# oxli-bio/oxli

Measured on NVIDIA B200. Metric: canonical k-mers counted/sec, higher is better.
Workload: dtype u64

## Files before the change

### oxli_b200/csrc/capi.cu

```cuda
#include <algorithm>
#include <atomic>
#include <cerrno>
#include <chrono>
#include <cmath>
#include <cstdarg>
#include <cstddef>
#include <condition_variable>
#include <cstdio>
#include <cstdlib>
#include <cstring>
#include <deque>
#include <functional>
#include <memory>
#include <mutex>
#include <string>
#include <system_error>
#include <thread>
#include <vector>

#include <fcntl.h>
#include <unistd.h>

#include <cuda_runtime.h>
#include <nvtx3/nvToolsExt.h>
// ... 205 lines not shown

constexpr uint64_t kScratchMin = 1024;

oxg_status ensure_io(DeviceCtx *c, uint64_t n) {
    CU(c->d_io.reserve(n, kScratchMin));
    CU(c->h_io.reserve(n, kScratchMin));
    return OXG_OK;
}

int grid_for(const DeviceCtx *c, uint64_t items, int threads, int per_sm) {
    uint64_t want = (items + threads - 1) / threads;
    return (int)std::max<uint64_t>(1, std::min<uint64_t>(want, (uint64_t)c->sms * per_sm));
}

constexpr uint64_t kSparseBytes = 128ull << 20;
uint64_t capacity_for_keys(uint64_t keys);
bool over_loaded(uint64_t size, uint64_t cap) {
    if (cap * 16 < kSparseBytes) return size * 10 > cap * 3;
    return size * 10 > cap * 7;
}

uint64_t pow2_at_least(uint64_t x) {
    uint64_t c = kMinCap;
    while (c < x) c <<= 1;
    return c;
}

uint64_t capacity_for_keys(uint64_t keys) {
    uint64_t cap = pow2_at_least(keys + keys / 2 + 1);
    while (cap * 16 < kSparseBytes && keys * 10 > cap * 3) cap <<= 1;
    return cap;
}

uint64_t slots_for(uint64_t keys) { return std::max(capacity_for_keys(keys), pow2_at_least(keys * 2)); }

oxg_status free_device_bytes(size_t *free_b) {
    size_t total = 0;
    CU(cudaMemGetInfo(free_b, &total));
    return OXG_OK;
}

oxg_status larger_and_fits(uint64_t keys, uint64_t cap, bool *yes) {
    *yes = false;
    const uint64_t want = slots_for(keys);
    if (want <= cap) return OXG_OK;
    size_t free_b = 0;
    TRY(free_device_bytes(&free_b));
    *yes = want * 16 < free_b / 2;
    return OXG_OK;
}


}

namespace {
struct PartPlan {
    uint32_t n_parts = 0, part_bits = 0;
    int n_ranks = 1, self_rank = 0, owner_shift = 64;
    uint32_t grid_a = 0;
    uint32_t frag_cap = 0;
    uint32_t batch_tiles = 1;
    uint64_t spill_cap = 0;
    uint32_t groups = 1;
    uint32_t n_dest() const { return n_parts * (uint32_t)n_ranks; }
    uint64_t frag_entries() const { return (uint64_t)n_dest() * grid_a * frag_cap; }
};

}

struct oxg_table {
    DeviceCtx *ctx = nullptr;
    uint32_t k = 0;
    DeviceArray<ulonglong2> slots;
    DeviceArray<Ctrl> d_ctrl;
    PinnedArray<Ctrl> h_ctrl;
    uint64_t size = 0;
    bool hinted = false;
    uint64_t hint_keys = 0;
    bool pooled = false;
    float last_ms_a = 0.f, last_ms_b = 0.f;
    struct {
        bool active = false;
        PartPlan pl;
        uint32_t launches = 0;
        uint64_t windows = 0, planned = 0;
    } pend;
    uint64_t part_budget = 0;
    uint32_t group_cap = 0;
    DeviceArray<uint32_t> d_sketch;
    PinnedArray<uint32_t> h_sketch;
    uint64_t sketch_covers = 0;
    uint64_t est_keys = 0;
    uint64_t last_made = 0;
    uint64_t last_new = 0;
    float last_ms = 0.f;
    uint64_t last_launches = 0;
};

namespace {

TableView view_of(const oxg_table *t, const DeferLists *defer = nullptr) {
    TableView v;
    v.slots = t->slots.get();
    v.cap = t->slots.cap();
    uint32_t lg = 0;
    while ((1ull << lg) < t->slots.cap()) ++lg;
    v.shift = 64 - lg;
    v.limit = t->slots.cap() - t->slots.cap() / 5;
    v.ctrl = t->d_ctrl.get();
    v.overflow = defer ? defer->pairs.get() : nullptr;
    v.overflow_cap = defer ? defer->pairs.cap() : 0;
    return v;
}

oxg_status pull_ctrl(oxg_table *t) {
    DeviceCtx *c = t->ctx;
    CU(cudaMemcpyAsync(t->h_ctrl.get(), t->d_ctrl.get(), sizeof(Ctrl), cudaMemcpyDeviceToHost, c->stream));
    CU(cudaStreamSynchronize(c->stream));
    t->size = t->h_ctrl.get()->size;
    return OXG_OK;
}

oxg_status zero_ctrl_fields(oxg_table *t, size_t first_field, size_t n_fields) {
    CU(cudaMemsetAsync(reinterpret_cast<uint64_t *>(t->d_ctrl.get()) + first_field, 0, n_fields * 8, t->ctx->stream));
    return OXG_OK;
}
constexpr size_t kFieldCounted = offsetof(Ctrl, counted) / 8;
constexpr size_t kFieldTile = offsetof(Ctrl, tile_counter) / 8;
constexpr size_t kLaunchFields = (offsetof(Ctrl, scratch) - offsetof(Ctrl, counted)) / 8;
constexpr size_t kFieldScratch = offsetof(Ctrl, scratch) / 8;

oxg_status alloc_slots(const oxg_table *t, uint64_t cap, DeviceArray<ulonglong2> *out) {
    DeviceCtx *c = t->ctx;
    if (t->pooled) *out = DeviceArray<ulonglong2>(c->stream);
    CU(out->reserve(cap));
    init_slots_kernel<<<grid_for(c, cap, kOpThreads, 16), kOpThreads, 0, c->stream>>>(out->get(), cap);
    LAUNCHED();
    CU(cudaGetLastError());
    return OXG_OK;
}

oxg_status grow_to_fit(oxg_table *t, uint64_t keys) {
    const uint64_t want = slots_for(keys);
    if (want <= t->slots.cap()) return OXG_OK;
    DeviceCtx *c = t->ctx;
    DeviceArray<ulonglong2> old;
    TRY(alloc_slots(t, want, &old));
    std::swap(t->slots, old);
    if (t->size) {
        rehash_kernel<<<grid_for(c, old.cap(), kOpThreads, 16), kOpThreads, 0, c->stream>>>(old.get(), old.cap(), view_of(t));
        LAUNCHED();
        CU(cudaGetLastError());
    }
    CU(cudaStreamSynchronize(c->stream));
    return OXG_OK;
}

oxg_status reserve_keys(oxg_table *t, uint64_t extra) { return grow_to_fit(t, t->size + extra); }

template <class Rebuild, class SideDrops>
oxg_status rebuild_slots(oxg_table *t, const Rebuild &rebuild, const SideDrops &side_drops, uint64_t *removed) {
    DeviceArray<ulonglong2> old;
    TRY(alloc_slots(t, t->slots.cap(), &old));
    std::swap(t->slots, old);
    rebuild(old.get());
    LAUNCHED();
    CU(cudaGetLastError());
    TRY(pull_ctrl(t));
    old.reset();
    Ctrl *h = t->h_ctrl.get();
    uint64_t n = h->scratch[0];
    h->size -= n;
    if (h->side_present && side_drops(h->side_count)) { h->side_present = 0; h->side_count = 0; ++n; }
    t->size = h->size;
    CU(cudaMemcpyAsync(t->d_ctrl.get(), h, offsetof(Ctrl, counted), cudaMemcpyHostToDevice, t->ctx->stream));
    CU(cudaStreamSynchronize(t->ctx->stream));
    if (removed) *removed = n;
    return OXG_OK;
}

oxg_status drain_deferred(oxg_table *t, DeferLists &d, uint64_t ov) {
    NvtxRange range("oxg:replay deferred");
    DeviceCtx *c = t->ctx;
    if (ov > d.pairs.cap()) return fail(OXG_ERR_CUDA, "internal: overflow list overrun");
    uint64_t prev = ~0ULL;
    while (ov) {
        const uint64_t room = std::min<uint64_t>(ov, std::max<uint64_t>(t->size, 1ull << 20));
        const uint64_t cap_before = t->slots.cap();
        TRY(grow_to_fit(t, t->size + room));
        const bool last = t->slots.cap() == cap_before && ov >= prev;
        if (last) TRY(grow_to_fit(t, t->size + ov));
        prev = ov;
        if (!last) {
            if (!d.fixed) CU(d.pairs2.reserve(ov, kScratchMin));
            else if (d.pairs2.cap() < ov) return fail(OXG_ERR_NOMEM, "deferral list too small for the replay");
        }
        TRY(zero_ctrl_fields(t, offsetof(Ctrl, overflow) / 8, 1));
        TableView v = view_of(t);
        if (!last) { v.overflow = d.pairs2.get(); v.overflow_cap = d.pairs2.cap(); }
        replay_pairs_kernel<<<grid_for(c, (ov + 3) / 4, kOpThreads, 8), kOpThreads, 0, c->stream>>>(v, d.pairs.get(), ov);
        LAUNCHED();
        CU(cudaGetLastError());
        TRY(pull_ctrl(t));
        ov = t->h_ctrl.get()->overflow;
        std::swap(d.pairs, d.pairs2);
    }
    return OXG_OK;
}

struct Counting { float ms = 0.f; uint64_t made = 0, ov = 0; };
oxg_status end_counting(oxg_table *t, uint64_t launches, uint64_t *counted, Counting *out) {
    DeviceCtx *c = t->ctx;
    CU(cudaEventRecord(c->ev_t1, c->stream));
    const uint64_t size_before = t->size;
    TRY(pull_ctrl(t));
    CU(cudaEventElapsedTime(&out->ms, c->ev_t0, c->ev_t1));
    t->last_ms += out->ms; t->last_launches += launches;
    if (counted) *counted += t->h_ctrl.get()->counted;
    out->made = t->size - size_before;
    out->ov = t->h_ctrl.get()->overflow;
    return OXG_OK;
}

#define OXG_DECLARE_ENTRY(KK) extern "C" const void *oxg_consume_entry_##KK(int mode);
OXG_FOR_EACH_K(OXG_DECLARE_ENTRY)
#undef OXG_DECLARE_ENTRY
const void *specialised_entry(uint32_t k, int mode) {
    switch (k) {
#define OXG_K_ENTRY(KK) case KK: return oxg_consume_entry_##KK(mode);
        OXG_FOR_EACH_K(OXG_K_ENTRY)
#undef OXG_K_ENTRY
    default:
        return nullptr;
    }
}
bool specialised_k(uint32_t k) { return specialised_entry(k, kModeCount) != nullptr; }
uint32_t tile_width(uint32_t k) { return specialised_k(k) ? kWarpTile : kTileW; }

oxg_status max_dyn_smem(const void *fn, int dev, size_t bytes) {
    static std::mutex mu;
    static std::vector<std::pair<const void *, int>> done;
    std::lock_guard<std::mutex> lk(mu);
    const std::pair<const void *, int> key{fn, dev};
    if (std::find(done.begin(), done.end(), key) != done.end()) return OXG_OK;
    CU(cudaFuncSetAttribute(fn, cudaFuncAttributeMaxDynamicSharedMemorySize, (int)bytes));
    done.push_back(key);
    return OXG_OK;
}

template <int MODE>
oxg_status launch_consume(oxg_table *t, const ConsumeParams &p) {
    DeviceCtx *c = t->ctx;
    const int k = (int)t->k;
    auto grid_of = [&](const void *fn, size_t smem) {
        int per_sm = 1;
        if (cudaOccupancyMaxActiveBlocksPerMultiprocessor(&per_sm, fn, kThreads, smem) != cudaSuccess || per_sm < 1) per_sm = 1;
        const uint64_t tiles_per_cta = specialised_k(t->k) ? kThreads / 32 : 1;
        const uint64_t work = p.n_tiles;
        return (int)std::max<uint64_t>(1, std::min<uint64_t>((work + tiles_per_cta - 1) / tiles_per_cta, (uint64_t)c->sms * per_sm));
    };
    if (const void *fn = specialised_entry(t->k, MODE)) {
        const size_t dyn = consume_dyn_smem(MODE);
        if (dyn) TRY(max_dyn_smem(fn, c->dev, dyn));
        void *args[] = {const_cast<ConsumeParams *>(&p)};
        CU(cudaLaunchKernel(fn, dim3(grid_of(fn, dyn)), dim3(kThreads), args, dyn, c->stream));
    } else {
        const size_t smem = generic_smem_bytes(k);
        consume_generic_kernel<MODE><<<grid_of((const void *)consume_generic_kernel<MODE>, smem), kThreads, smem, c->stream>>>(p);
    }
    LAUNCHED();
    CU(cudaGetLastError());
    return OXG_OK;
}



uint32_t group_launches(const oxg_table *t) {
    const uint32_t g = g_accumulate.load();
    return t->group_cap ? std::min(g, t->group_cap) : g;
}

bool use_partitioned(const oxg_table *t, uint64_t span) {
    if (!specialised_entry(t->k, kModePart)) return false;
    const int choice = g_pipeline.load();
    if (choice == 1) return false;
    if (choice == 2) return true;
    if (t->pend.active) return true;
    return span >= kPartMinWindows;
}

uint32_t choose_parts(const oxg_table *t, uint32_t max_parts) {
    const uint32_t forced = g_parts_override.load();
    if (forced >= 2 && !(forced & (forced - 1))) return std::min(forced, std::max(max_parts, 2u));
    const uint64_t est = std::max(t->size + t->last_new, t->hint_keys);
    if (est == 0) return std::min<uint32_t>(1024, max_parts);
    uint64_t parts = 64;
    while (parts < max_parts && parts * 6144 < est) parts <<= 1;
    return (uint32_t)std::min<uint64_t>(parts, max_parts);
}

size_t scatter_smem_rt(uint32_t k, uint32_t n_dest, uint32_t batch_tiles) {
    const uint32_t q = 8 * ((k + 7 + 7) / 8);
    const uint32_t bl = ((kWarpTile - 8 + q) + 15) / 16 * 16;
    return scatter_smem_bytes(n_dest, batch_tiles, (int)(2 * bl + 128));
}

uint64_t scatter_full_grid_tiles(const DeviceCtx *c) { return (uint64_t)c->sms * kScatCtasPerSm * kScatWarps; }
uint32_t scatter_grid(const DeviceCtx *c, uint64_t n_tiles) {
    return (uint32_t)std::max<uint64_t>(1, std::min<uint64_t>((n_tiles + kScatWarps - 1) / kScatWarps, (uint64_t)c->sms * kScatCtasPerSm));
}

oxg_status plan_partitioned(oxg_table *t, uint64_t span, uint64_t n_tiles, int n_ranks, int self_rank, PartPlan *out) {
    DeviceCtx *c = t->ctx;
    PartPlan pl;
    pl.n_parts = choose_parts(t, std::max(2u, 2048u / (uint32_t)n_ranks));
    while ((1u << pl.part_bits) < pl.n_parts) ++pl.part_bits;
    pl.n_ranks = n_ranks; pl.self_rank = self_rank;
    int lg = 0;
    while ((1 << lg) < n_ranks) ++lg;
    pl.owner_shift = 64 - lg;
    pl.batch_tiles = kScatMaxBatchTiles;
    while (pl.batch_tiles > 1 && scatter_smem_rt(t->k, pl.n_dest(), pl.batch_tiles) * kScatCtasPerSm > 220u * 1024) --pl.batch_tiles;
    if (scatter_smem_rt(t->k, pl.n_dest(), pl.batch_tiles) * kScatCtasPerSm > 220u * 1024) return fail(OXG_ERR_INVALID, "internal: too many scatter destinations");
    pl.grid_a = scatter_grid(c, n_tiles);
    if (pl.grid_a * (uint64_t)kMaxSources > kAggMaxFrags) return fail(OXG_ERR_INVALID, "internal: more pass A CTAs than pass B can take");
    const uint64_t fair = span / ((uint64_t)pl.n_dest() * pl.grid_a) + 1;
    uint64_t sq = 1;
    while (sq * sq < fair) ++sq;
    pl.frag_cap = (uint32_t)((fair + fair / 2 + 4 * sq + 3) & ~(uint64_t)3);
    pl.spill_cap = span;
    const uint32_t forced_groups = g_groups_override.load();
    pl.groups = forced_groups ? forced_groups : std::max<uint32_t>(1, std::min<uint32_t>(8, (4u * (uint32_t)c->sms + pl.n_parts - 1) / pl.n_parts));
    if (pl.frag_entries() >> 32) return fail(OXG_ERR_INVALID, "internal: fragment buffer too large for one launch");
    *out = pl;
    return OXG_OK;
}

oxg_status scatter_attr(DeviceCtx *c, uint32_t k) { return max_dyn_smem(specialised_entry(k, kModePart), c->dev, 227 * 1024); }

oxg_status ensure_part_buffers(DeviceCtx *c, const PartPlan &pl) {
    CU(c->d_frag.reserve(pl.frag_entries(), kScratchMin));
    CU(c->d_frag_cnt.reserve((uint64_t)pl.n_dest() * pl.grid_a, kScratchMin));
    CU(c->d_spill.reserve(pl.spill_cap, kScratchMin));
    CU(c->d_spill_n.reserve(1));
    return OXG_OK;
}

oxg_status launch_part_a(oxg_table *t, ConsumeParams p, const PartPlan &pl, uint64_t *d_frag, uint32_t *d_frag_cnt,
                         uint64_t *d_spill, unsigned long long *d_spill_n, cudaStream_t stream, bool append = false) {
    DeviceCtx *c = t->ctx;
    const void *fn = specialised_entry(t->k, kModePart);
    TRY(scatter_attr(c, t->k));
    const size_t dyn = scatter_smem_rt(t->k, pl.n_dest(), pl.batch_tiles);
    p.frag = d_frag; p.frag_cnt = d_frag_cnt; p.frag_cap = pl.frag_cap;
    p.n_parts = pl.n_parts; p.part_shift = 64 - pl.part_bits; p.n_dest = pl.n_dest(); p.batch_tiles = pl.batch_tiles;
    p.n_ranks = pl.n_ranks; p.self_rank = pl.self_rank; p.owner_shift = pl.owner_shift;
    p.spill = d_spill; p.spill_cap = pl.spill_cap; p.spill_n = d_spill_n;
    p.frag_append = append ? 1u : 0u;
    if (p.n_tiles >> 31) return fail(OXG_ERR_INVALID, "internal: too many tiles for one pass A launch");
    if (!append) CU(cudaMemsetAsync(d_spill_n, 0, 8, stream));
    void *args[] = {&p};
    CU(cudaLaunchKernel(fn, dim3(pl.grid_a), dim3(kScatThreads), args, dyn, stream));
    LAUNCHED();
    CU(cudaGetLastError());
    return OXG_OK;
}

constexpr int kAggThreadsDirect = 1024;
const void *const kAggCached = (const void *)aggregate_kernel<kAggThreadsDefault, true>;
const void *const kAggDirect = (const void *)aggregate_kernel<kAggThreadsDirect, false>;

uint32_t use_cache_for(const oxg_table *t, const PartPlan &pl, uint64_t windows) {
    const uint64_t keys = std::max(std::max(t->size, t->hint_keys), t->est_keys);
    return keys == 0 || (windows >= 2 * keys && keys <= 8192ull * pl.n_parts) ? 1u : 0u;
}

uint32_t aggregate_groups(const PartPlan &pl, uint32_t use_cache, uint64_t hashes) {
    if (use_cache || g_groups_override.load()) return pl.groups;
    const uint64_t items = std::max<uint64_t>(1, hashes / 40960);
    return (uint32_t)std::max<uint64_t>(pl.groups, std::min<uint64_t>(64, (items + pl.n_parts - 1) / pl.n_parts));
}

AggParams agg_params(const TableView &v, const PartPlan &pl, const AggSource *src, int n_src) {
    AggParams a{};
    a.table = v;
    for (int s = 0; s < n_src; ++s) a.src[s] = src[s];
    a.n_src = n_src;
    a.n_parts = pl.n_parts; a.dest0 = (uint32_t)pl.self_rank * pl.n_parts; a.n_ctas = pl.grid_a;
    a.frag_cap = pl.frag_cap; a.part_bits = pl.part_bits; a.spill_cap = pl.spill_cap;
    a.owner_shift = pl.owner_shift; a.self_rank = pl.self_rank; a.n_ranks = pl.n_ranks;
    return a;
}

oxg_status launch_part_b(oxg_table *t, const TableView &v, const PartPlan &pl, const AggSource *src, int n_src,
                         uint64_t windows, cudaStream_t stream) {
    DeviceCtx *c = t->ctx;
    AggParams a = agg_params(v, pl, src, n_src);
    a.work_counter = (unsigned long long *)&t->d_ctrl.get()->absorb_counter;
    a.use_cache = use_cache_for(t, pl, windows);
    a.groups = aggregate_groups(pl, a.use_cache, windows);
    const void *fn = a.use_cache ? kAggCached : kAggDirect;
    const int threads = a.use_cache ? kAggThreadsDefault : kAggThreadsDirect;
    const size_t smem = aggregate_smem_bytes(a.use_cache != 0);
    if (a.use_cache) TRY(max_dyn_smem(fn, c->dev, smem));
    int per_sm = 1;
    if (cudaOccupancyMaxActiveBlocksPerMultiprocessor(&per_sm, fn, threads, smem) != cudaSuccess || per_sm < 1) per_sm = 1;
    const uint64_t items = (uint64_t)a.n_parts * a.groups;
    const int grid = (int)std::max<uint64_t>(1, std::min<uint64_t>(items, (uint64_t)c->sms * per_sm));
    void *args[] = {&a};
    CU(cudaLaunchKernel(fn, dim3(grid), dim3(threads), args, smem, stream));
    LAUNCHED();
    CU(cudaGetLastError());
    return OXG_OK;
}

oxg_status ensure_sketch(oxg_table *t, cudaStream_t st) {
    if (t->h_sketch.get()) return OXG_OK;
    CU(t->d_sketch.reserve(kSketchRegs));
    CU(cudaMemsetAsync(t->d_sketch.get(), 0, kSketchRegs * 4, st));
    CU(t->h_sketch.reserve(kSketchRegs));
    return OXG_OK;
}

double sketch_estimate(const uint32_t *regs) {
    const double m = (double)kSketchRegs;
    double sum = 0.0;
    uint32_t zeros = 0;
    for (uint32_t i = 0; i < kSketchRegs; ++i) { sum += std::ldexp(1.0, -(int)regs[i]); zeros += regs[i] == 0; }
    const double alpha = 0.7213 / (1.0 + 1.079 / m);
    double e = alpha * m * m / sum;
    if (e <= 2.5 * m && zeros) e = m * std::log(m / (double)zeros);
    return e;
}

oxg_status presize_for_group(oxg_table *t, const PartPlan &pl, const AggSource *src, int n_src, cudaStream_t stream,
                             uint64_t arrivals = 0, uint64_t rounds_left = 1) {
    DeviceCtx *c = t->ctx;
    TRY(ensure_sketch(t, stream));
    sketch_kernel<<<c->sms * 2, 512, 0, stream>>>(agg_params(TableView{}, pl, src, n_src), t->d_sketch.get());
    LAUNCHED();
    CU(cudaGetLastError());
    CU(cudaMemcpyAsync(t->h_sketch.get(), t->d_sketch.get(), kSketchRegs * 4, cudaMemcpyDeviceToHost, stream));
    CU(cudaStreamSynchronize(stream));
    const uint64_t unseen = t->size > t->sketch_covers ? t->size - t->sketch_covers : 0;
    const double est = sketch_estimate(t->h_sketch.get());
    t->est_keys = (uint64_t)est + unseen;
    double headroom = 1.0;
    if (rounds_left > 1) headroom = est * 4 >= (double)arrivals ? std::max(4.0, 0.5 * (double)rounds_left) : (double)std::min<uint64_t>(4, rounds_left);
    uint64_t expect = (uint64_t)(est * 1.04 * headroom) + unseen + 1024;
    if (headroom > 4.0) {
        size_t free_b = 0;
        TRY(free_device_bytes(&free_b));
        while (headroom > 4.0 && slots_for(expect) * 16 > free_b / 2) {
            headroom /= 2;
            expect = (uint64_t)(est * 1.04 * std::max(headroom, 4.0)) + unseen + 1024;
        }
    }
    if (expect * 10 > t->slots.cap() * 7) TRY(grow_to_fit(t, expect));
    return OXG_OK;
}

oxg_status flush_pending(oxg_table *t, uint64_t *counted) {
    if (!t->pend.active) return OXG_OK;
    NvtxRange range("oxg:aggregate (pass B)");
    DeviceCtx *c = t->ctx;
    t->pend.active = false;
    CU(cudaEventRecord(c->ev_mid, c->stream));
    const AggSource own{c->d_frag.get(), c->d_frag_cnt.get(), c->d_spill.get(), c->d_spill_n.get()};
    const bool hint_holds = t->hinted && t->size <= t->hint_keys;
    const bool roomy = t->size != 0 && (t->size + 2 * t->last_made) * 10 <= t->slots.cap() * 7;
    const bool sketched = !hint_holds && !roomy;
    if (sketched) TRY(presize_for_group(t, t->pend.pl, &own, 1, c->stream));
    TRY(launch_part_b(t, view_of(t, &c->defer), t->pend.pl, &own, 1, t->pend.windows, c->stream));
    Counting r;
    TRY(end_counting(t, t->pend.launches, counted, &r));
    float ms_a = 0.f;
    CU(cudaEventElapsedTime(&ms_a, c->ev_t0, c->ev_mid));
    t->last_ms_a += ms_a; t->last_ms_b += r.ms - ms_a;
    const uint64_t made = r.made;
    t->last_new = r.ov ? made + r.ov : (t->hinted && t->size <= t->hint_keys) ? 0 : made;
    if (r.ov) TRY(drain_deferred(t, c->defer, r.ov));
    t->last_made = made;
    if (sketched) t->sketch_covers = t->size;
    if (!hint_holds) {
        if (made * 4 >= t->pend.windows && t->part_budget && t->size * 20 >= t->slots.cap() * 7) {
            const uint64_t more = (uint64_t)((double)made / (double)t->pend.windows * 0.6 * (double)t->part_budget);
            const uint64_t want = t->size + more;
            bool grow = false;
            TRY(larger_and_fits(want, t->slots.cap(), &grow));
            if (grow) TRY(grow_to_fit(t, want));
        }
    }
    return OXG_OK;
}

oxg_status run_span(oxg_table *t, int mode, const uint8_t *d_bases, uint64_t g0, uint64_t w_lo,
                    uint64_t w_hi, uint64_t data_end, const uint64_t *d_offsets, uint64_t n_off,
                    uint64_t *hashes_out, uint64_t *counted) {
    DeviceCtx *c = t->ctx;
    if (w_hi <= w_lo) return OXG_OK;
    if ((reinterpret_cast<uintptr_t>(d_bases) & 15) || (g0 & 15))
        return fail(OXG_ERR_INVALID, "device base buffer must be 16-byte aligned");
    uint64_t lo = w_lo;
    while (lo < w_hi) {
        const uint64_t tile_base = std::max<uint64_t>(g0, lo & ~(uint64_t)15);
        uint64_t hi = std::min<uint64_t>(w_hi, tile_base + kLaunchWindows);
        const uint32_t tw = tile_width(t->k);
        const uint64_t n_tiles = (hi - tile_base + tw - 1) / tw;
        CU(c->d_tile_first.reserve(n_tiles, kScratchMin));
        if (mode == kModeCount) {
            const uint64_t span = hi - lo;
            if (t->pend.active && !use_partitioned(t, span)) TRY(flush_pending(t, counted));
            if (span <= kSmallBatch) TRY(reserve_keys(t, span));
            else {
                if (!t->hinted && t->slots.cap() < pow2_at_least(span / 8)) TRY(grow_to_fit(t, span / 16));
                const uint64_t expect = t->size + t->last_new + t->last_new / 4;
                if (expect * 10 > t->slots.cap() * 7) TRY(grow_to_fit(t, expect));
                else if (over_loaded(t->size, t->slots.cap())) TRY(grow_to_fit(t, t->size));
            }
            CU(c->defer.pairs.reserve(std::max<uint64_t>(span, t->pend.active ? t->pend.planned : 0), kScratchMin));
            if (!t->pend.active) TRY(zero_ctrl_fields(t, kFieldCounted, kLaunchFields));
        } else {
            TRY(zero_ctrl_fields(t, kFieldTile, 1));
        }
        ConsumeParams p{};
        p.bases = d_bases; p.g0 = g0; p.w_lo = lo; p.w_hi = hi; p.data_end = data_end;
        p.tile_base = tile_base; p.n_tiles = n_tiles; p.offsets = d_offsets; p.n_off = n_off;
        p.tile_first = c->d_tile_first.get(); p.table = view_of(t, mode == kModeCount ? &c->defer : nullptr);
        p.hashes_out = hashes_out ? hashes_out + (lo - w_lo) : nullptr; p.ksize = t->k;
        tile_first_kernel<<<(unsigned)((n_tiles + 255) / 256), 256, 0, c->stream>>>(d_offsets, n_off, tile_base, n_tiles, tw, c->d_tile_first.get());
        LAUNCHED();
        CU(cudaGetLastError());
        const bool part = mode == kModeCount && use_partitioned(t, hi - lo);
        if (part) {
            NvtxRange range("oxg:scatter (pass A)");
            const uint64_t span = hi - lo;
            if (t->pend.active && t->pend.windows + span > t->pend.planned) TRY(flush_pending(t, counted));
            if (!t->pend.active) {
                const uint64_t planned = std::min<uint64_t>(std::max<uint64_t>(t->part_budget, span), (uint64_t)group_launches(t) * kLaunchWindows);
                TRY(plan_partitioned(t, planned, planned / tw + 1, 1, 0, &t->pend.pl));
                TRY(ensure_part_buffers(c, t->pend.pl));
                t->pend.active = true; t->pend.launches = 0; t->pend.windows = 0; t->pend.planned = planned;
                CU(cudaEventRecord(c->ev_t0, c->stream));
            }
            TRY(launch_part_a(t, p, t->pend.pl, c->d_frag.get(), c->d_frag_cnt.get(), c->d_spill.get(), c->d_spill_n.get(), c->stream, t->pend.launches > 0));
            t->pend.launches += 1; t->pend.windows += span;
            t->part_budget = t->part_budget > span ? t->part_budget - span : 0;
            if (t->pend.launches >= group_launches(t) || t->pend.windows >= t->pend.planned) TRY(flush_pending(t, counted));
            lo = hi;
            continue;
        }
        NvtxRange range(mode == kModeCount ? "oxg:consume (fused)" : mode == kModeHash ? "oxg:hash windows" : "oxg:first-bad scan");
        CU(cudaEventRecord(c->ev_t0, c->stream));
        if (mode == kModeCount) TRY(launch_consume<kModeCount>(t, p));
        else if (mode == kModeHash) TRY(launch_consume<kModeHash>(t, p));
        else TRY(launch_consume<kModeFirstBad>(t, p));
        if (mode == kModeCount) {
            Counting r;
            TRY(end_counting(t, 1, counted, &r));
            t->last_new = (hi - lo) <= kSmallBatch ? 0 : r.ov ? r.made + r.ov : 4 * t->h_ctrl.get()->late_new;
            if (r.ov) TRY(drain_deferred(t, c->defer, r.ov));
        }
        lo = hi;
    }
    return OXG_OK;
}


template <class Span>
oxg_status first_bad_window(oxg_table *t, const Span &span, uint64_t n_win, uint64_t total, uint64_t *fb) {
    t->h_ctrl.get()->first_bad = ~0ULL;
    CU(cudaMemcpyAsync(&t->d_ctrl.get()->first_bad, &t->h_ctrl.get()->first_bad, 8, cudaMemcpyHostToDevice, t->ctx->stream));
    TRY(span(kModeFirstBad, 0, n_win, total, nullptr));
    TRY(pull_ctrl(t));
    *fb = t->h_ctrl.get()->first_bad;
    return OXG_OK;
}

oxg_status read_of(DeviceCtx *c, const uint64_t *h_offsets, const uint64_t *d_offsets, uint64_t n_reads, uint64_t fb,
                   uint64_t *r, uint64_t *r_start) {
    std::vector<uint64_t> tmp;
    uint64_t base0 = 0;
    if (h_offsets) {
        base0 = h_offsets[0];
    } else {
        tmp.resize(n_reads + 1);
        CU(cudaMemcpyAsync(tmp.data(), d_offsets, (n_reads + 1) * 8, cudaMemcpyDeviceToHost, c->stream));
        CU(cudaStreamSynchronize(c->stream));
        h_offsets = tmp.data();
    }
    *r = (uint64_t)(std::upper_bound(h_offsets, h_offsets + n_reads + 1, base0 + fb) - h_offsets) - 1;
    *r_start = h_offsets[*r] - base0;
    return OXG_OK;
}

oxg_status bad_kmer(uint64_t r, uint64_t pos, int64_t *err_read, uint64_t *err_pos) {
    if (err_read) *err_read = (int64_t)r;
    if (err_pos) *err_pos = pos;
    return fail(OXG_ERR_BAD_KMER, "bad k-mer encountered at position %llu", (unsigned long long)pos);
}

template <class Span>
oxg_status consume_batch(oxg_table *t, const Span &span, const uint64_t *h_offsets, const uint64_t *d_offsets,
                         uint64_t n_reads, uint64_t total, int skip_bad, uint32_t group_cap,
                         uint64_t *total_counted, int64_t *err_read, uint64_t *err_pos) {
    const uint64_t k = t->k;
    if (total_counted) *total_counted = 0;
// ... 888 lines not shown
```

### oxli_b200/csrc/scatter.cuh

```cuda
#pragma once
#include "consume.cuh"

namespace oxg {

#ifndef OXG_SCAT_THREADS
#define OXG_SCAT_THREADS 384
#endif
#ifndef OXG_SCAT_CTAS
#define OXG_SCAT_CTAS 2
#endif
constexpr int kScatThreads = OXG_SCAT_THREADS;
constexpr int kScatCtasPerSm = OXG_SCAT_CTAS;
constexpr int kScatWarps = kScatThreads / 32;
constexpr int kScatMaxBatchTiles = 3;
static_assert(kScatWarps * 256 >= 2048, "step 2 scans 256 destinations per warp, up to 2048 of them");

template <int K>
struct ScatWarpBuf {
    static constexpr int BL = TileGeom<K>::BL;
    static constexpr int kBytes = 2 * BL + 64 + 64;
};

__host__ __device__ inline size_t scatter_dest_bytes(uint32_t n_dest) { return ((size_t)n_dest * 12 + 15) & ~(size_t)15; }
__host__ __device__ inline size_t scatter_smem_bytes(uint32_t n_dest, uint32_t batch_tiles, int warp_buf_bytes) {
    return (size_t)kScatWarps * batch_tiles * kWarpTile * 8 + scatter_dest_bytes(n_dest) + 16 + (size_t)kScatWarps * warp_buf_bytes;
}

template <int K>
__global__ void __launch_bounds__(kScatThreads, kScatCtasPerSm) scatter_kernel(const ConsumeParams p) {
    using G = TileGeom<K>;
    constexpr int BL = G::BL, NV = G::NV, NE = G::NE;
    constexpr int kMaxPerLane = kScatMaxBatchTiles * kWPT;
    static_assert(NV + 8 <= 32 && NE <= 16, "per-warp mask buffers are 64 bytes each");
    extern __shared__ __align__(128) uint8_t sm[];
    const int lane = threadIdx.x & 31, warp = threadIdx.x >> 5;
    const uint32_t nd = p.n_dest, slice = p.batch_tiles * kWarpTile;
    uint64_t *batch = reinterpret_cast<uint64_t *>(sm);
    uint32_t *cnt = reinterpret_cast<uint32_t *>(batch + (size_t)kScatWarps * slice);
    uint32_t *pos = cnt + nd, *to_frag = pos + nd;
    uint32_t *s_total = reinterpret_cast<uint32_t *>(reinterpret_cast<uint8_t *>(cnt) + scatter_dest_bytes(nd));
    unsigned long long *s_counted = reinterpret_cast<unsigned long long *>(s_total + 2);
    uint8_t *wbuf = reinterpret_cast<uint8_t *>(s_total + 4) + (size_t)warp * ScatWarpBuf<K>::kBytes;
    uint8_t *s_fw = wbuf, *s_rc = wbuf + BL;
    uint16_t *s_bad = reinterpret_cast<uint16_t *>(wbuf + 2 * BL);
    uint32_t *s_end = reinterpret_cast<uint32_t *>(wbuf + 2 * BL + 64);
    uint64_t *const my_slice = batch + (size_t)warp * slice;

    const uint32_t frag_row = gridDim.x * p.frag_cap;
    uint64_t *const my_frag = p.frag + (uint64_t)blockIdx.x * p.frag_cap;
    for (uint32_t i = threadIdx.x; i < nd; i += kScatThreads) {
        to_frag[i] = p.frag_append ? p.frag_cnt[(uint64_t)i * gridDim.x + blockIdx.x] : 0u;
        cnt[i] = 0; pos[i] = 0;
    }
    if (threadIdx.x == 0) *s_counted = 0;
    __syncthreads();

    auto dest_of = [&](uint64_t h) {
        uint32_t d = (uint32_t)((h * kPhi) >> p.part_shift);
        if (p.n_ranks > 1) d += (uint32_t)(h >> p.owner_shift) * p.n_parts;
        return d;
    };

    uint64_t first_bad_unused = ~0ULL;
    const uint32_t n_tiles = (uint32_t)p.n_tiles, tiles_per_round = gridDim.x * kScatWarps;
    const uint32_t n_rounds = (n_tiles + tiles_per_round - 1) / tiles_per_round;
    const uint32_t R = p.batch_tiles, n_batches = (n_rounds + R - 1) / R;
    auto tile_of = [&](uint32_t r) { return (r * gridDim.x + blockIdx.x) * kScatWarps + warp; };

    uint4 raw = make_uint4(0, 0, 0, 0);
    uint64_t tf = 0, off = ~0ULL;
    auto fetch = [&](uint32_t t, uint4 &raw_, uint64_t &tf_) {
        if (t < n_tiles) {
            if (lane < NV) raw_ = load_bases16(p, p.tile_base + (uint64_t)t * kWarpTile + 16ull * lane);
            tf_ = __ldg(p.tile_first + t);
        }
    };
    auto fetch_off = [&](uint32_t t, uint64_t tf_) {
        const uint64_t rr = tf_ + lane;
        return (t < n_tiles && rr < p.n_off) ? __ldg(p.offsets + rr) : ~0ULL;
    };
    fetch(tile_of(0), raw, tf);
    off = fetch_off(tile_of(0), tf);

    for (uint32_t b = 0; b < n_batches; ++b) {
        const uint32_t r0 = b * R, n_here = min(r0 + R, n_rounds) - r0;

        for (uint32_t i = 0; i < n_here; ++i) {
            const uint32_t r = r0 + i, t = tile_of(r);
            uint4 raw_next = make_uint4(0, 0, 0, 0);
            uint64_t tf_next = 0;
            fetch(tile_of(r + 1), raw_next, tf_next);
            uint64_t h[kWPT] = {};
            if (t < n_tiles) {
                const uint64_t w0 = p.tile_base + (uint64_t)t * kWarpTile;
                if (lane < NE) s_end[lane] = 0;
                __syncwarp();
                if (lane < NV) stage16_raw<BL>(p, w0, lane, raw, s_fw, s_rc, s_bad);
                {
                    const uint64_t e = off - 1 - w0;
                    if (e < (uint64_t)BL) atomicOr(&s_end[e >> 5], 1u << (e & 31));
                    if (__shfl_sync(0xffffffffu, e < (uint64_t)BL, 31)) {
                        for (uint64_t q = tf + 32 + lane; q < p.n_off; q += 32) {
                            const uint64_t e2 = p.offsets[q] - 1 - w0;
                            if (e2 >= (uint64_t)BL) break;
                            atomicOr(&s_end[e2 >> 5], 1u << (e2 & 31));
                        }
                    }
                }
                __syncwarp();
                const uint32_t valid = lane_valid_mask<K, kModePart>(p, s_bad, s_end, w0, lane, first_bad_unused);
                if (valid) lane_hashes<K>(s_fw, s_rc, lane * kWPT, valid, h);
            }
            off = fetch_off(tile_of(r + 1), tf_next);
            raw = raw_next; tf = tf_next;
#pragma unroll
            for (int j = 0; j < kWPT; ++j) {
                if (h[j] != 0) atomicAdd(&cnt[dest_of(h[j])], 1u);
                my_slice[i * kWarpTile + j * 32 + lane] = h[j];
            }
            __syncwarp();
        }
        __syncthreads();

        if (warp * 256u < nd) {
            const uint32_t lo = warp * 256u;
            uint32_t carry = 0;
            for (uint32_t d = lane; d < lo; d += 32) carry += cnt[d];
            carry = __reduce_add_sync(0xffffffffu, carry);
            uint32_t v[8], x[8];
#pragma unroll
            for (int u = 0; u < 8; ++u) {
                const uint32_t d = lo + 32 * u + lane;
                v[u] = d < nd ? cnt[d] : 0u;
                x[u] = v[u];
            }
#pragma unroll
            for (int o = 1; o < 32; o <<= 1) {
#pragma unroll
                for (int u = 0; u < 8; ++u) {
                    const uint32_t y = __shfl_up_sync(0xffffffffu, x[u], o);
                    if (lane >= o) x[u] += y;
                }
            }
#pragma unroll
            for (int u = 0; u < 8; ++u) {
                const uint32_t d = lo + 32 * u + lane;
                if (d < nd) {
                    const uint32_t start = carry + x[u] - v[u], fill = min(to_frag[d] + pos[d], p.frag_cap);
                    pos[d] = start; to_frag[d] = fill - start;
                }
                carry += __shfl_sync(0xffffffffu, x[u], 31);
            }
            if (lane == 0 && lo + 256u >= nd) { *s_total = carry; *s_counted += carry; }
        }
        uint64_t v[kMaxPerLane];
#pragma unroll
        for (int u = 0; u < kMaxPerLane; ++u) v[u] = u < (int)(n_here * kWPT) ? my_slice[u * 32 + lane] : 0ull;
        __syncthreads();

        for (uint32_t d = threadIdx.x; d < nd; d += kScatThreads) cnt[d] = 0;
#pragma unroll
        for (int u = 0; u < kMaxPerLane; ++u)
            if (v[u] != 0) batch[atomicAdd(&pos[dest_of(v[u])], 1u)] = v[u];
        __syncthreads();

        const uint32_t total = *s_total;
        for (uint32_t i0 = warp * 128; i0 < total; i0 += kScatThreads * 4) {
            uint64_t h[4];
#pragma unroll
            for (int u = 0; u < 4; ++u) {
                const uint32_t i = i0 + 32 * u + lane;
                h[u] = i < total ? batch[i] : 0ull;
            }
            uint32_t spilled = 0;
#pragma unroll
            for (int u = 0; u < 4; ++u) {
                if (h[u] == 0) continue;
                const uint32_t d = dest_of(h[u]), at = i0 + 32 * u + lane + to_frag[d];
                if (at < p.frag_cap) my_frag[d * frag_row + at] = h[u];
                else spilled |= 1u << u;
            }
            if (__any_sync(0xffffffffu, spilled != 0)) {
                const uint32_t mine = __popc(spilled);
                uint32_t incl = mine;
                for (int o = 1; o < 32; o <<= 1) {
                    const uint32_t y = __shfl_up_sync(0xffffffffu, incl, o);
                    if (lane >= o) incl += y;
                }
                unsigned long long base = 0;
                if (lane == 31) base = atomicAdd(p.spill_n, (unsigned long long)incl);
                base = __shfl_sync(0xffffffffu, base, 31) + (incl - mine);
#pragma unroll
                for (int u = 0; u < 4; ++u)
                    if ((spilled >> u) & 1u) { if (base < p.spill_cap) p.spill[base] = h[u]; ++base; }
            }
        }
        __syncthreads();
    }

    for (uint32_t d = threadIdx.x; d < nd; d += kScatThreads)
        p.frag_cnt[(uint64_t)d * gridDim.x + blockIdx.x] = min(to_frag[d] + pos[d], p.frag_cap);
    if (threadIdx.x == 0 && *s_counted) atomicAdd((unsigned long long *)&p.table.ctrl->counted, *s_counted);
}

}
```

Measured before the change: 42.84 billion.

## Compact valid lanes into a slot queue before hashing in scatter kernel

Adds a per-warp slot queue that records only lanes that have valid k-mer windows, with tiles double-buffered in shared memory. Hashing then runs over densely packed 32-lane rounds instead of sparse per-tile rounds, which cuts divergence and wasted lanes when many windows are invalid. Per-destination counts and positions shrink to packed 16-bit counters updated through 32-bit atomics, saving shared memory. The cost is more complex control flow, a larger per-warp buffer, and batch termination now decided by __syncthreads_or.

```diff
diff --git a/oxli_b200/csrc/capi.cu b/oxli_b200/csrc/capi.cu
--- a/oxli_b200/csrc/capi.cu
+++ b/oxli_b200/csrc/capi.cu
@@ -531,7 +531,7 @@
 size_t scatter_smem_rt(uint32_t k, uint32_t n_dest, uint32_t batch_tiles) {
     const uint32_t q = 8 * ((k + 7 + 7) / 8);
     const uint32_t bl = ((kWarpTile - 8 + q) + 15) / 16 * 16;
-    return scatter_smem_bytes(n_dest, batch_tiles, (int)(2 * bl + 128));
+    return scatter_smem_bytes(n_dest, batch_tiles, scatter_warp_buf_bytes((int)bl));
 }
 
 uint64_t scatter_full_grid_tiles(const DeviceCtx *c) { return (uint64_t)c->sms * kScatCtasPerSm * kScatWarps; }
diff --git a/oxli_b200/csrc/scatter.cuh b/oxli_b200/csrc/scatter.cuh
--- a/oxli_b200/csrc/scatter.cuh
+++ b/oxli_b200/csrc/scatter.cuh
@@ -1,5 +1,6 @@
 #pragma once
 #include "consume.cuh"
+#include "slot_queue.h"
 
 namespace oxg {
 
@@ -14,14 +15,15 @@
 constexpr int kScatWarps = kScatThreads / 32;
 constexpr int kScatMaxBatchTiles = 3;
 static_assert(kScatWarps * 256 >= 2048, "step 2 scans 256 destinations per warp, up to 2048 of them");
-
+static_assert(kScatWarps * kScatMaxBatchTiles * kWarpTile < 65536, "counts and run positions of a batch fit 16 bits");
+
+__host__ __device__ constexpr int scatter_warp_buf_bytes(int bl) { return 4 * bl + 64 + 64 + (int)kSlotQueueCap * 2; }
 template <int K>
 struct ScatWarpBuf {
-    static constexpr int BL = TileGeom<K>::BL;
-    static constexpr int kBytes = 2 * BL + 64 + 64;
+    static constexpr int kBytes = scatter_warp_buf_bytes(TileGeom<K>::BL);
 };
 
-__host__ __device__ inline size_t scatter_dest_bytes(uint32_t n_dest) { return ((size_t)n_dest * 12 + 15) & ~(size_t)15; }
+__host__ __device__ inline size_t scatter_dest_bytes(uint32_t n_dest) { return ((size_t)n_dest * 8 + 15) & ~(size_t)15; }
 __host__ __device__ inline size_t scatter_smem_bytes(uint32_t n_dest, uint32_t batch_tiles, int warp_buf_bytes) {
     return (size_t)kScatWarps * batch_tiles * kWarpTile * 8 + scatter_dest_bytes(n_dest) + 16 + (size_t)kScatWarps * warp_buf_bytes;
 }
@@ -36,14 +38,15 @@
     const int lane = threadIdx.x & 31, warp = threadIdx.x >> 5;
     const uint32_t nd = p.n_dest, slice = p.batch_tiles * kWarpTile;
     uint64_t *batch = reinterpret_cast<uint64_t *>(sm);
-    uint32_t *cnt = reinterpret_cast<uint32_t *>(batch + (size_t)kScatWarps * slice);
-    uint32_t *pos = cnt + nd, *to_frag = pos + nd;
-    uint32_t *s_total = reinterpret_cast<uint32_t *>(reinterpret_cast<uint8_t *>(cnt) + scatter_dest_bytes(nd));
+    uint32_t *to_frag = reinterpret_cast<uint32_t *>(batch + (size_t)kScatWarps * slice);
+    uint16_t *cnt = reinterpret_cast<uint16_t *>(to_frag + nd), *pos = cnt + nd;
+    uint32_t *cnt2 = reinterpret_cast<uint32_t *>(cnt), *pos2 = reinterpret_cast<uint32_t *>(pos);
+    uint32_t *s_total = reinterpret_cast<uint32_t *>(reinterpret_cast<uint8_t *>(to_frag) + scatter_dest_bytes(nd));
     unsigned long long *s_counted = reinterpret_cast<unsigned long long *>(s_total + 2);
     uint8_t *wbuf = reinterpret_cast<uint8_t *>(s_total + 4) + (size_t)warp * ScatWarpBuf<K>::kBytes;
-    uint8_t *s_fw = wbuf, *s_rc = wbuf + BL;
-    uint16_t *s_bad = reinterpret_cast<uint16_t *>(wbuf + 2 * BL);
-    uint32_t *s_end = reinterpret_cast<uint32_t *>(wbuf + 2 * BL + 64);
+    uint16_t *s_bad = reinterpret_cast<uint16_t *>(wbuf + 4 * BL);
+    uint32_t *s_end = reinterpret_cast<uint32_t *>(wbuf + 4 * BL + 64);
+    uint16_t *s_queue = reinterpret_cast<uint16_t *>(wbuf + 4 * BL + 128);
     uint64_t *const my_slice = batch + (size_t)warp * slice;
 
     const uint32_t frag_row = gridDim.x * p.frag_cap;
@@ -62,45 +65,47 @@
     };
 
     uint64_t first_bad_unused = ~0ULL;
-    const uint32_t n_tiles = (uint32_t)p.n_tiles, tiles_per_round = gridDim.x * kScatWarps;
-    const uint32_t n_rounds = (n_tiles + tiles_per_round - 1) / tiles_per_round;
-    const uint32_t R = p.batch_tiles, n_batches = (n_rounds + R - 1) / R;
+    const uint32_t n_tiles = (uint32_t)p.n_tiles, R = p.batch_tiles;
     auto tile_of = [&](uint32_t r) { return (r * gridDim.x + blockIdx.x) * kScatWarps + warp; };
 
     uint4 raw = make_uint4(0, 0, 0, 0);
-    uint64_t tf = 0, off = ~0ULL;
+    uint64_t tf = 0;
     auto fetch = [&](uint32_t t, uint4 &raw_, uint64_t &tf_) {
         if (t < n_tiles) {
             if (lane < NV) raw_ = load_bases16(p, p.tile_base + (uint64_t)t * kWarpTile + 16ull * lane);
             tf_ = __ldg(p.tile_first + t);
         }
     };
-    auto fetch_off = [&](uint32_t t, uint64_t tf_) {
+    auto fetch_end = [&](uint32_t t, uint64_t tf_) {
         const uint64_t rr = tf_ + lane;
-        return (t < n_tiles && rr < p.n_off) ? __ldg(p.offsets + rr) : ~0ULL;
+        if (t >= n_tiles || rr >= p.n_off) return ~0u;
+        return (uint32_t)min(__ldg(p.offsets + rr) - 1 - (p.tile_base + (uint64_t)t * kWarpTile), (uint64_t)~0u);
     };
     fetch(tile_of(0), raw, tf);
-    off = fetch_off(tile_of(0), tf);
-
-    for (uint32_t b = 0; b < n_batches; ++b) {
-        const uint32_t r0 = b * R, n_here = min(r0 + R, n_rounds) - r0;
-
-        for (uint32_t i = 0; i < n_here; ++i) {
-            const uint32_t r = r0 + i, t = tile_of(r);
-            uint4 raw_next = make_uint4(0, 0, 0, 0);
-            uint64_t tf_next = 0;
-            fetch(tile_of(r + 1), raw_next, tf_next);
-            uint64_t h[kWPT] = {};
-            if (t < n_tiles) {
+    uint32_t end = fetch_end(tile_of(0), tf);
+    bool end_stale = false;
+    SlotQueue sq;
+
+    bool more;
+    do {
+        sq.new_batch();
+        while (sq.rounds() < R) {
+            const uint32_t t = tile_of(sq.staged);
+            if (sq.may_stage(t < n_tiles)) {
+                const uint32_t b = sq.next_buffer();
+                uint8_t *s_fw = wbuf + 2 * BL * b, *s_rc = s_fw + BL;
+                if (end_stale) end = fetch_end(t, __ldg(p.tile_first + t));
+                uint4 raw_next = make_uint4(0, 0, 0, 0);
+                uint64_t tf_next = 0;
+                fetch(tile_of(sq.staged + 1), raw_next, tf_next);
                 const uint64_t w0 = p.tile_base + (uint64_t)t * kWarpTile;
                 if (lane < NE) s_end[lane] = 0;
                 __syncwarp();
                 if (lane < NV) stage16_raw<BL>(p, w0, lane, raw, s_fw, s_rc, s_bad);
                 {
-                    const uint64_t e = off - 1 - w0;
-                    if (e < (uint64_t)BL) atomicOr(&s_end[e >> 5], 1u << (e & 31));
-                    if (__shfl_sync(0xffffffffu, e < (uint64_t)BL, 31)) {
-                        for (uint64_t q = tf + 32 + lane; q < p.n_off; q += 32) {
+                    if (end < (uint32_t)BL) atomicOr(&s_end[end >> 5], 1u << (end & 31));
+                    if (__shfl_sync(0xffffffffu, end < (uint32_t)BL, 31)) {
+                        for (uint64_t q = __ldg(p.tile_first + t) + 32 + lane; q < p.n_off; q += 32) {
                             const uint64_t e2 = p.offsets[q] - 1 - w0;
                             if (e2 >= (uint64_t)BL) break;
                             atomicOr(&s_end[e2 >> 5], 1u << (e2 & 31));
@@ -109,18 +114,36 @@
                 }
                 __syncwarp();
                 const uint32_t valid = lane_valid_mask<K, kModePart>(p, s_bad, s_end, w0, lane, first_bad_unused);
-                if (valid) lane_hashes<K>(s_fw, s_rc, lane * kWPT, valid, h);
-            }
-            off = fetch_off(tile_of(r + 1), tf_next);
-            raw = raw_next; tf = tf_next;
-#pragma unroll
-            for (int j = 0; j < kWPT; ++j) {
-                if (h[j] != 0) atomicAdd(&cnt[dest_of(h[j])], 1u);
-                my_slice[i * kWarpTile + j * 32 + lane] = h[j];
+                const uint32_t queued = __ballot_sync(0xffffffffu, valid != 0);
+                if (valid)
+                    s_queue[(sq.tail() + __popc(queued & ((1u << lane) - 1))) % kSlotQueueCap] =
+                        (uint16_t)(b << 13 | (uint32_t)lane << 8 | valid);
+                sq.stage(__popc(queued));
+                raw = raw_next; tf = tf_next; end_stale = true;
+            } else if (sq.queued() != 0) {
+                const uint32_t n = sq.round_size(), i = sq.rounds();
+                const uint32_t e = (uint32_t)lane < n ? s_queue[(sq.head() + lane) % kSlotQueueCap] : 0u;
+                end = fetch_end(t, tf); end_stale = false;
+                sq.round(n);
+                uint64_t h[kWPT] = {};
+                if (e != 0) {
+                    const uint8_t *s_fw = wbuf + 2 * BL * (e >> 13);
+                    lane_hashes<K>(s_fw, s_fw + BL, (int)((e >> 8) & 31) * kWPT, e & 0xffu, h);
+                }
+#pragma unroll
+                for (int j = 0; j < kWPT; ++j) {
+                    if (h[j] != 0) {
+                        const uint32_t d = dest_of(h[j]);
+                        atomicAdd(&cnt2[d >> 1], 1u << (16 * (d & 1)));
+                    }
+                    my_slice[i * kWarpTile + j * 32 + lane] = h[j];
+                }
+            } else {
+                break;
             }
             __syncwarp();
         }
-        __syncthreads();
+        more = __syncthreads_or(tile_of(sq.staged) < n_tiles || sq.queued() != 0);
 
         if (warp * 256u < nd) {
             const uint32_t lo = warp * 256u;
@@ -155,13 +178,16 @@
         }
         uint64_t v[kMaxPerLane];
 #pragma unroll
-        for (int u = 0; u < kMaxPerLane; ++u) v[u] = u < (int)(n_here * kWPT) ? my_slice[u * 32 + lane] : 0ull;
+        for (int u = 0; u < kMaxPerLane; ++u) v[u] = u < (int)(sq.rounds() * kWPT) ? my_slice[u * 32 + lane] : 0ull;
         __syncthreads();
 
         for (uint32_t d = threadIdx.x; d < nd; d += kScatThreads) cnt[d] = 0;
 #pragma unroll
         for (int u = 0; u < kMaxPerLane; ++u)
-            if (v[u] != 0) batch[atomicAdd(&pos[dest_of(v[u])], 1u)] = v[u];
+            if (v[u] != 0) {
+                const uint32_t d = dest_of(v[u]), sh = 16 * (d & 1);
+                batch[(atomicAdd(&pos2[d >> 1], 1u << sh) >> sh) & 0xffffu] = v[u];
+            }
         __syncthreads();
 
         const uint32_t total = *s_total;
@@ -196,7 +222,7 @@
             }
         }
         __syncthreads();
-    }
+    } while (more);
 
     for (uint32_t d = threadIdx.x; d < nd; d += kScatThreads)
         p.frag_cnt[(uint64_t)d * gridDim.x + blockIdx.x] = min(to_frag[d] + pos[d], p.frag_cap);
diff --git a/oxli_b200/csrc/slot_queue.h b/oxli_b200/csrc/slot_queue.h
--- /dev/null
+++ b/oxli_b200/csrc/slot_queue.h
@@ -0,0 +1,37 @@
+#pragma once
+#include <cstdint>
+
+#if defined(__CUDACC__)
+#define OXG_HD __host__ __device__ __forceinline__
+#else
+#define OXG_HD inline
+#endif
+
+namespace oxg {
+
+constexpr uint32_t kSlotQueueCap = 64;
+
+struct SlotQueue {
+    uint32_t staged = 0;
+    uint32_t w = 0;
+
+    OXG_HD uint32_t queued() const { return w & 0xffu; }
+    OXG_HD uint32_t head() const { return (w >> 8) & 0xffu; }
+    OXG_HD uint32_t tail() const { return (head() + queued()) % kSlotQueueCap; }
+    OXG_HD uint32_t older() const { return (w >> 16) & 0xffu; }
+    OXG_HD uint32_t rounds() const { return w >> 24; }
+    OXG_HD uint32_t next_buffer() const { return staged & 1u; }
+    OXG_HD void new_batch() { w &= 0xffffffu; }
+    OXG_HD bool may_stage(bool tile_left) const { return tile_left && queued() < 32 && older() == 0; }
+    OXG_HD void stage(uint32_t n_slots) {
+        w = (w & 0xff00ff00u) | queued() << 16 | (queued() + n_slots);
+        ++staged;
+    }
+    OXG_HD uint32_t round_size() const { return queued() < 32 ? queued() : 32u; }
+    OXG_HD void round(uint32_t n) {
+        const uint32_t old = older() > n ? older() - n : 0u;
+        w = (rounds() + 1) << 24 | old << 16 | ((head() + n) % kSlotQueueCap) << 8 | (queued() - n);
+    }
+};
+
+}
```

New measurement: 44.24 billion (median of 6 runs). 3.3% higher.
